# SYSTRAN/faster-whisper

Hardware: AMD Instinct MI355X
Metric: audio-sec/sec (RTF) large-v3 fp16 beam=5 batch=16 (higher is better)
Workload: dtype f16

## Files before the change

faster_whisper_amd/csrc/dec_kernels.hip:

```cpp
#include "common.h"
#include "dec_kernels.h"
#include <stdlib.h>
#include <atomic>
#include <type_traits>

namespace fwd {
static std::atomic<int> g_self_attn_form{0};
static std::atomic<int> g_forms_epoch{0};
static std::atomic<int> g_cross_regs{0};
}

__device__ __forceinline__ size_t frag_off(int row, int k, int KS) {
  return ((size_t)((row >> 4) * KS + (k >> 5)) * 64 + ((k >> 3) & 3) * 16 + (row & 15)) * 8 + (k & 7);
}

static __device__ __forceinline__ int ragged_pos(const int* __restrict__ ptab, int chunk, int step, int reach) {
  const int p = ptab[chunk] - 1 + step;
  return p < reach ? p : reach - 1;
}

__global__ void dec_embed_kernel(const int* __restrict__ tok, const half_t* __restrict__ emb,
                                 const half_t* __restrict__ pos_emb, half_t* __restrict__ x,
                                 half_t* __restrict__ xfrag, int d, const int* __restrict__ d_step, int pos_fixed,
                                 int P, int blk_n, const int* __restrict__ ptab, int kmul, int reach) {
// ... 621 lines not shown
    int rt = rt0 + a; if (rt > n_rt - 1) rt = n_rt - 1;
    xp[a] = reinterpret_cast<const intx4*>(xfv) + (size_t)rt * KS * 64 + lane;
  }
  floatx4 accf[RT][NT];
  intx4 acci[RT][NT];
  float rs[RT], rq[RT];
#pragma unroll
  for (int a = 0; a < RT; ++a) {
    rs[a] = 0.f; rq[a] = 0.f;
#pragma unroll
    for (int b = 0; b < NT; ++b) { accf[a][b] = floatx4{0, 0, 0, 0}; acci[a][b] = intx4{0, 0, 0, 0}; }
  }
  struct Set { intx4 w[CH][NT]; intx4 x[CH][RT]; };
  auto load = [&](Set& f, int ks0) {
#pragma unroll
    for (int j = 0; j < CH; ++j) {
      int ks = ks0 + j; if (ks > KS - 1) ks = KS - 1;
#pragma unroll
      for (int b = 0; b < NT; ++b) f.w[j][b] = wp[b][(size_t)ks * 64];
#pragma unroll
      for (int a = 0; a < RT; ++a) f.x[j][a] = xp[a][(size_t)ks * 64];
    }
  };
  auto compute = [&](const Set& f, int ks0) {
#pragma unroll
    for (int j = 0; j < CH; ++j) {
      if (ks0 + j < KS) {
#pragma unroll
        for (int a = 0; a < RT; ++a) {
#pragma unroll
          for (int b = 0; b < NT; ++b) {
            if (I8) acci[a][b] = __builtin_amdgcn_mfma_i32_16x16x64_i8(f.w[j][b], f.x[j][a], acci[a][b], 0, 0, 0);
            else accf[a][b] = __builtin_amdgcn_mfma_f32_16x16x32_f16(__builtin_bit_cast(half8_t, f.w[j][b]),
                                                                    __builtin_bit_cast(half8_t, f.x[j][a]), accf[a][b],
                                                                    0, 0, 0);
          }
          if (LNF && !SPLIT) {
            const half8_t xv = __builtin_bit_cast(half8_t, f.x[j][a]);
            const half2_t one2 = {(half_t)1.f, (half_t)1.f};
#pragma unroll
            for (int e = 0; e < 4; ++e) {
              const half2_t h2 = {xv[2 * e], xv[2 * e + 1]};
              rs[a] = __builtin_amdgcn_fdot2(h2, one2, rs[a], false);
              rq[a] = __builtin_amdgcn_fdot2(h2, h2, rq[a], false);
            }
          }
        }
        if (SPLIT) {
          const half2_t one2 = {(half_t)1.f, (half_t)1.f};
          const intx4 xsel = wn == 0 ? f.x[j][0] : (wn == 1 ? f.x[j][1] : (wn == 2 ? f.x[j][2] : f.x[j][RT > 3 ? 3 : 0]));
          const half8_t xv = __builtin_bit_cast(half8_t, xsel);
#pragma unroll
          for (int e = 0; e < 4; ++e) {
            const half2_t h2 = {xv[2 * e], xv[2 * e + 1]};
            rs[0] = __builtin_amdgcn_fdot2(h2, one2, rs[0], false);
            rq[0] = __builtin_amdgcn_fdot2(h2, h2, rq[0], false);
          }
          if (RT > 4 && wn == 0) {
            const half8_t xw = __builtin_bit_cast(half8_t, f.x[j][RT > 4 ? 4 : 0]);
#pragma unroll
            for (int e = 0; e < 4; ++e) {
              const half2_t h2 = {xw[2 * e], xw[2 * e + 1]};
              rs[1] = __builtin_amdgcn_fdot2(h2, one2, rs[1], false);
              rq[1] = __builtin_amdgcn_fdot2(h2, h2, rq[1], false);
            }
          }
        }
      }
    }
  };
  float ks1[NT][4], kcf[NT][4], kws[NT][4];
  half_t kb[NT][4];
#pragma unroll
  for (int b = 0; b < NT; ++b) {
#pragma unroll
    for (int e = 0; e < 4; ++e) {
      const int n = (ct0 + b) * 16 + 4 * g + e;
      const int ne = n < N ? n : N - 1;
      ks1[b][e] = kcf[b][e] = 0.f; kws[b][e] = 1.f; kb[b][e] = (half_t)0.f;
      if (I8) kws[b][e] = w_scale[ne];
      if (LNF) { ks1[b][e] = s1[ne]; kcf[b][e] = cf[ne]; }
      else if (bias) kb[b][e] = bias[ne];
    }
  }
  Set fa, fb;
  load(fa, 0);
  for (int ks0 = 0; ks0 < KS; ks0 += 2 * CH) {
    load(fb, ks0 + CH);
    compute(fa, ks0);
    load(fa, ks0 + 2 * CH);
    compute(fb, ks0 + CH);
  }
  if (SPLIT) {
#pragma unroll
    for (int q = 0; q < 2; ++q) {
      if (q == 1 && !(RT > 4 && wn == 0)) break;
      float sa = rs[q], sb = rq[q];
      sa += __shfl_xor(sa, 16, 64); sa += __shfl_xor(sa, 32, 64);
      sb += __shfl_xor(sb, 16, 64); sb += __shfl_xor(sb, 32, 64);
      if (g == 0) { xst[q == 0 ? wn : 4][i][0] = sa; xst[q == 0 ? wn : 4][i][1] = sb; }
    }
    __syncthreads();
  }
#pragma unroll
  for (int a = 0; a < RT; ++a) {
    float mu = 0.f, rstd = 1.f;
    if (LNF) {
      float sa, sb;
      if (SPLIT) {
        sa = xst[a][i][0]; sb = xst[a][i][1];
      } else {
        sa = rs[a]; sb = rq[a];
        sa += __shfl_xor(sa, 16, 64); sa += __shfl_xor(sa, 32, 64);
        sb += __shfl_xor(sb, 16, 64); sb += __shfl_xor(sb, 32, 64);
      }
      mu = sa / (float)K;
      rstd = rsqrtf(fmaxf(sb / (float)K - mu * mu, 0.f) + 1e-5f);
    }
    const int row = (rt0 + a) * 16 + i;
    if (rt0 + a >= n_rt || row >= R) continue;
    const float sx = I8 ? x_scale[row] : 1.f;
    const bool pair_ok = (ldo & 1) == 0;
#pragma unroll
    for (int b = 0; b < NT; ++b) {
      if (ct0 + b >= n_ct) continue;
      const int n = (ct0 + b) * 16 + 4 * g;
      float t4[4];
#pragma unroll
      for (int e = 0; e < 4; ++e) {
        float tv = I8 ? (float)acci[a][b][e] * sx * kws[b][e] : accf[a][b][e];
        if (LNF) tv = rstd * (tv - mu * ks1[b][e]) + kcf[b][e];
        else if (bias) tv += (float)kb[b][e];
        t4[e] = tv;
      }
      if (F32 && pair_ok) {
        float* o = reinterpret_cast<float*>(outv) + (size_t)row * ldo + n;
        if (n + 1 < N) *reinterpret_cast<floatx2*>(o) = floatx2{t4[0], t4[1]};
        else if (n < N) o[0] = t4[0];
        if (n + 3 < N) *reinterpret_cast<floatx2*>(o + 2) = floatx2{t4[2], t4[3]};
        else if (n + 2 < N) o[2] = t4[2];
        continue;
      }
#pragma unroll
      for (int e = 0; e < 4; ++e) {
        if (n + e >= N) continue;
        if (F32) reinterpret_cast<float*>(outv)[(size_t)row * ldo + n + e] = t4[e];
        else reinterpret_cast<half_t*>(outv)[(size_t)row * ldo + n + e] = (half_t)t4[e];
      }
    }
  }
}

#define SA_MAX_CTX 448
static __device__ __forceinline__ float sum8_dpp(float v) {
  v += __builtin_bit_cast(float, __builtin_amdgcn_update_dpp(0, __builtin_bit_cast(int, v), 0xB1, 0xF, 0xF, true));
  v += __builtin_bit_cast(float, __builtin_amdgcn_update_dpp(0, __builtin_bit_cast(int, v), 0x4E, 0xF, 0xF, true));
  v += __builtin_bit_cast(float, __builtin_amdgcn_update_dpp(0, __builtin_bit_cast(int, v), 0x141, 0xF, 0xF, true));
  return v;
}
template <bool RAG = false>
__global__ __launch_bounds__(1024) __attribute__((amdgpu_waves_per_eu(8, 8))) void dec_self_attn_kernel(const half_t* __restrict__ qkv, int d, half_t* __restrict__ kc,
                                                             half_t* __restrict__ vc, int n_ctx, int cache_ctx,
                                                             int H, const uint8_t* __restrict__ kvidx2, int Kbeam, int kmul,
                                                             half_t* __restrict__ out, const int* __restrict__ d_step,
                                                             int pos_fixed, int P, int R_total, int frag,
                                                             const int* __restrict__ ptab, int reach) {
  extern __shared__ float sa_smem[];
  const int lane = threadIdx.x & 63;
  const int wave = __builtin_amdgcn_readfirstlane(threadIdx.x >> 6);
  float* sp = sa_smem + (size_t)wave * 2 * n_ctx;
  int* ssrc = reinterpret_cast<int*>(sp + n_ctx);
  const int h = blockIdx.x, c = blockIdx.y;
  const int r = c * kmul + wave, kb = wave;
  const int step = *d_step;
  const int pos = RAG ? ragged_pos(ptab, c, step, reach) : (pos_fixed >= 0 ? pos_fixed : P - 1 + step);
  const int slot = c * Kbeam + kb;
  const int cur = (pos_fixed >= 0) ? 0 : (step & 1);
  const uint8_t* kvidx = kvidx2 + ((size_t)cur * R_total + slot) * n_ctx;
  const half_t* qr = qkv + (size_t)r * 3 * d + h * 64;
  const size_t head_stride = (size_t)cache_ctx * 64;
  const size_t slot_stride = (size_t)H * head_stride;
  const int pg = lane >> 3, cc = lane & 7;
  const half8_t q8 = *reinterpret_cast<const half8_t*>(qr + cc * 8);
  const half8_t kn8 = *reinterpret_cast<const half8_t*>(qr + d + cc * 8);
  const half8_t vn8 = *reinterpret_cast<const half8_t*>(qr + 2 * d + cc * 8);
  float q[8];
#pragma unroll
  for (int e = 0; e < 8; ++e) q[e] = (float)q8[e] * 0.125f;
  if (pg == 0) {
    *reinterpret_cast<half8_t*>(kc + slot * slot_stride + h * head_stride + (size_t)pos * 64 + cc * 8) = kn8;
    *reinterpret_cast<half8_t*>(vc + slot * slot_stride + h * head_stride + (size_t)pos * 64 + cc * 8) = vn8;
  }
  auto dot8 = [&](const half8_t& k) {
    float sacc = 0.f;
#pragma unroll
    for (int e = 0; e < 8; ++e) sacc += q[e] * (float)k[e];
    return sum8_dpp(sacc);
  };
  const float s_new = dot8(kn8);
  float mx = s_new;
  const half_t* kbase = kc + h * head_stride + cc * 8;
  for (int p0 = 0; p0 < pos; p0 += 32) {
    half8_t kv[4];
    int src[4];
#pragma unroll
    for (int j = 0; j < 4; ++j) {
      const int p = p0 + 8 * j + pg;
      const int pc = p < pos ? p : pos - 1;
      src[j] = c * Kbeam + kvidx[pc];
      kv[j] = *reinterpret_cast<const half8_t*>(kbase + src[j] * slot_stride + (size_t)pc * 64);
    }
#pragma unroll
    for (int j = 0; j < 4; ++j) {
      const int p = p0 + 8 * j + pg;
      const float sc = dot8(kv[j]);
      if (p < pos) {
        if (cc == 0) { sp[p] = sc; ssrc[p] = src[j]; }
        mx = fmaxf(mx, sc);
      }
    }
  }
  mx = wave_max(mx);
  __builtin_amdgcn_wave_barrier();
  float sum = 0.f;
  for (int p = lane; p < pos; p += 64) {
    const float e = __expf(sp[p] - mx);
    sp[p] = e;
    sum += e;
  }
  const float e_new = __expf(s_new - mx);
  sum = wave_sum(sum) + e_new;
  __builtin_amdgcn_wave_barrier();
  float acc[8];
#pragma unroll
  for (int e = 0; e < 8; ++e) acc[e] = 0.f;
  const half_t* vb = vc + h * head_stride + cc * 8;
#pragma unroll 4
  for (int p = pg; p < pos; p += 8) {
    const half8_t vv = *reinterpret_cast<const half8_t*>(vb + ssrc[p] * slot_stride + (size_t)p * 64);
    const float w = sp[p];
#pragma unroll
    for (int e = 0; e < 8; ++e) acc[e] += w * (float)vv[e];
  }
#pragma unroll
  for (int e = 0; e < 8; ++e) {
    float a = acc[e];
    a += __shfl_xor(a, 8, 64);
    a += __shfl_xor(a, 16, 64);
    a += __shfl_xor(a, 32, 64);
    acc[e] = a;
  }
  if (pg == 0) {
    const float inv = 1.f / sum;
    half8_t o;
#pragma unroll
    for (int e = 0; e < 8; ++e) o[e] = (half_t)((acc[e] + e_new * (float)vn8[e]) * inv);
    half_t* dst = frag ? out + frag_off(r, h * 64 + cc * 8, d >> 5) : out + (size_t)r * d + h * 64 + cc * 8;
    *reinterpret_cast<half8_t*>(dst) = o;
  }
}

template <int U, bool PIPE, int MAXT, bool PB = false, bool RAG = false>
__global__ __launch_bounds__(MAXT) void dec_self_attn2_kernel(const half_t* __restrict__ qkv, int d, half_t* __restrict__ kc,
                                                             half_t* __restrict__ vc, int n_ctx, int cache_ctx,
                                                             int H, const uint8_t* __restrict__ kvidx2, int Kbeam, int kmul,
                                                             half_t* __restrict__ out, const int* __restrict__ d_step,
                                                             int pos_fixed, int P, int R_total, int frag,
                                                             const int* __restrict__ ptab, int reach) {
  static_assert(!(PB && RAG), "position blocks take explicit positions");
  extern __shared__ float sa_smem[];
  constexpr int NB = 4 * U;
  const int lane = threadIdx.x & 63;
  const int wave = __builtin_amdgcn_readfirstlane(threadIdx.x >> 6);
  float* sp = sa_smem + (size_t)wave * 2 * n_ctx;
  int* ssrc = reinterpret_cast<int*>(sp + n_ctx);
  const int h = blockIdx.x, c = blockIdx.y;
  const int r = c * kmul + wave, kb = PB ? 0 : wave;
  const int step = PB ? 0 : *d_step;
  const int pos = PB ? pos_fixed + wave
                     : (RAG ? ragged_pos(ptab, c, step, reach) : (pos_fixed >= 0 ? pos_fixed : P - 1 + step));
  const int slot = c * Kbeam + kb;
  const int cur = (pos_fixed >= 0) ? 0 : (step & 1);
  const uint8_t* kvidx = kvidx2 + ((size_t)cur * R_total + slot) * n_ctx;
  const half_t* qr = qkv + (size_t)r * 3 * d + h * 64;
  const size_t head_stride = (size_t)cache_ctx * 64;
  const size_t slot_stride = (size_t)H * head_stride;
  const int pg = lane >> 3, cc = lane & 7;
  for (int p4 = 4 * lane; p4 < pos; p4 += 256) {
    const unsigned w = PB ? 0u : *reinterpret_cast<const unsigned*>(kvidx + p4);
    intx4 s4;
    s4[0] = c * Kbeam + (int)(w & 0xffu); s4[1] = c * Kbeam + (int)((w >> 8) & 0xffu);
    s4[2] = c * Kbeam + (int)((w >> 16) & 0xffu); s4[3] = c * Kbeam + (int)(w >> 24);
    *reinterpret_cast<intx4*>(ssrc + p4) = s4;
  }
  const half8_t q8 = *reinterpret_cast<const half8_t*>(qr + cc * 8);
  const half8_t kn8 = *reinterpret_cast<const half8_t*>(qr + d + cc * 8);
  const half8_t vn8 = *reinterpret_cast<const half8_t*>(qr + 2 * d + cc * 8);
  float q[8];
#pragma unroll
  for (int e = 0; e < 8; ++e) q[e] = (float)q8[e] * 0.125f;
  if (pg == 0) {
    *reinterpret_cast<half8_t*>(kc + slot * slot_stride + h * head_stride + (size_t)pos * 64 + cc * 8) = kn8;
    *reinterpret_cast<half8_t*>(vc + slot * slot_stride + h * head_stride + (size_t)pos * 64 + cc * 8) = vn8;
  }
  auto dot8 = [&](const half8_t& k) {
    float sacc = 0.f;
#pragma unroll
    for (int e = 0; e < 8; ++e) sacc = __builtin_fmaf(q[e], (float)k[e], sacc);
    return sum8_dpp(sacc);
  };
  const float s_new = dot8(kn8);
  float mx = s_new;
  __builtin_amdgcn_wave_barrier();
  const char* kbase = reinterpret_cast<const char*>(kc + h * head_stride);
  const char* vbase = reinterpret_cast<const char*>(vc + h * head_stride);
  const unsigned slot_bytes = (unsigned)(slot_stride * sizeof(half_t));
  struct Batch { half8_t row[NB]; };
  auto fetch = [&](Batch& b, const char* base, int p0, const half_t* sib) {
#pragma unroll
    for (int j = 0; j < NB; ++j) {
      const int p = p0 + 8 * j + pg;
      const int pc = p < pos ? p : pos - 1;
      const unsigned off = (unsigned)ssrc[pc] * slot_bytes + (unsigned)(pc * 128 + cc * 16);
      if (PB && pc >= pos_fixed)
        b.row[j] = *reinterpret_cast<const half8_t*>(sib + (size_t)(pc - pos_fixed) * 3 * d + cc * 8);
      else
        b.row[j] = *reinterpret_cast<const half8_t*>(base + off);
    }
  };
  const half_t* ksib = qkv + (size_t)c * kmul * 3 * d + d + h * 64;
  const half_t* vsib = ksib + d;
  auto score = [&](const Batch& b, int p0) {
#pragma unroll
    for (int j = 0; j < NB; ++j) {
      const int p = p0 + 8 * j + pg;
      const float sc = dot8(b.row[j]);
      if (p < pos) {
        if (cc == 0) sp[p] = sc;
        mx = fmaxf(mx, sc);
      }
    }
  };
  Batch b0, b1;
  if (pos > 0) {
    fetch(b0, kbase, 0, ksib);
    for (int p0 = 0; p0 < pos; p0 += 16 * NB) {
      if (PIPE) {
        fetch(b1, kbase, p0 + 8 * NB, ksib);
        score(b0, p0);
        fetch(b0, kbase, p0 + 16 * NB, ksib);
        score(b1, p0 + 8 * NB);
      } else {
        score(b0, p0);
        if (p0 + 8 * NB < pos) {
          fetch(b0, kbase, p0 + 8 * NB, ksib);
          score(b0, p0 + 8 * NB);
          if (p0 + 16 * NB < pos) fetch(b0, kbase, p0 + 16 * NB, ksib);
        }
      }
    }
    fetch(b0, vbase, 0, vsib);
  }
  mx = wave_max_v(mx);
  __builtin_amdgcn_wave_barrier();
  float sum = 0.f;
  for (int p = lane; p < pos; p += 64) {
    const float e = __expf(sp[p] - mx);
    sp[p] = e;
    sum += e;
  }
  const float e_new = __expf(s_new - mx);
  sum = wave_sum_v(sum) + e_new;
  __builtin_amdgcn_wave_barrier();
  float acc[8];
#pragma unroll
  for (int e = 0; e < 8; ++e) acc[e] = 0.f;
  auto accum = [&](const Batch& b, int p0) {
#pragma unroll
    for (int j = 0; j < NB; ++j) {
      const int p = p0 + 8 * j + pg;
      if (p < pos) {
        const float w = sp[p];
#pragma unroll
        for (int e = 0; e < 8; ++e) acc[e] = __builtin_fmaf(w, (float)b.row[j][e], acc[e]);
      }
    }
  };
  for (int p0 = 0; p0 < pos; p0 += 16 * NB) {
    if (PIPE) {
      fetch(b1, vbase, p0 + 8 * NB, vsib);
      accum(b0, p0);
      fetch(b0, vbase, p0 + 16 * NB, vsib);
      accum(b1, p0 + 8 * NB);
    } else {
      accum(b0, p0);
      if (p0 + 8 * NB < pos) {
        fetch(b0, vbase, p0 + 8 * NB, vsib);
        accum(b0, p0 + 8 * NB);
        if (p0 + 16 * NB < pos) fetch(b0, vbase, p0 + 16 * NB, vsib);
      }
    }
  }
#pragma unroll
  for (int e = 0; e < 8; ++e) acc[e] = sum_x8_x16_x32_v(acc[e]);
  if (pg == 0) {
    const float inv = 1.f / sum;
    half8_t o;
#pragma unroll
    for (int e = 0; e < 8; ++e) o[e] = (half_t)((acc[e] + e_new * (float)vn8[e]) * inv);
    half_t* dst = frag ? out + frag_off(r, h * 64 + cc * 8, d >> 5) : out + (size_t)r * d + h * 64 + cc * 8;
    *reinterpret_cast<half8_t*>(dst) = o;
  }
}

template <int CA_WAVES, bool NTL, int MINW = 1>
__global__ __launch_bounds__(CA_WAVES * 64, MINW) void dec_cross_attn_kernel(const half_t* __restrict__ qx, int d,
                                                             const half_t* __restrict__ ck,
                                                             const half_t* __restrict__ cvt, int T, int kvp,
                                                             int kmul, half_t* __restrict__ out,
                                                             const int* __restrict__ done, int kv_div, int frag,
                                                             const int* __restrict__ slot_map) {
  __shared__ float sm[CA_WAVES][16], sl[CA_WAVES][16];
  __shared__ float so[CA_WAVES][16][65];
  const int h = blockIdx.x, c = blockIdx.y;
  if (done && done[c]) return;
  const int tid = threadIdx.x, lane = tid & 63, wave = tid >> 6;
  const int j = lane & 15, g = lane >> 4;
  const int ce = slot_map[c / kv_div];
  const half_t* kbase = ck + ((size_t)ce * (d >> 6) + h) * kvp * 64 + lane * 8;
  const half_t* vbase = cvt + ((size_t)ce * (d >> 6) + h) * kvp * 64 + lane * 8;
  half8_t qf[2];
  {
    if (j < kmul) {
      const half_t* qp = qx + (size_t)(c * kmul + j) * d + h * 64 + g * 8;
#pragma unroll
      for (int s = 0; s < 2; ++s) {
        half8_t v = *reinterpret_cast<const half8_t*>(qp + s * 32);
#pragma unroll
        for (int e = 0; e < 8; ++e) v[e] = v[e] * (half_t)0.125f;
        qf[s] = v;
      }
    } else {
      qf[0] = half8_t{0, 0, 0, 0, 0, 0, 0, 0};
      qf[1] = qf[0];
    }
  }
  floatx4 o[4];
#pragma unroll
  for (int dt = 0; dt < 4; ++dt) o[dt] = floatx4{0, 0, 0, 0};
  float m_run = -1.0e30f, l_run = 0.f;
  const float LOG2E = 1.4426950408889634f;
  const int ngroups = (T + 31) >> 5;
  auto load_kv = [&](int gi, half8_t (&kf)[4], half8_t (&vf)[4]) {
    const half_t* kp = kbase + (size_t)gi * 2048;
    const half_t* vp = vbase + (size_t)gi * 2048;
#pragma unroll
    for (int q = 0; q < 4; ++q)
      kf[q] = NTL ? __builtin_nontemporal_load(reinterpret_cast<const half8_t*>(kp + q * 512))
                  : *reinterpret_cast<const half8_t*>(kp + q * 512);
#pragma unroll
    for (int dt = 0; dt < 4; ++dt)
      vf[dt] = NTL ? __builtin_nontemporal_load(reinterpret_cast<const half8_t*>(vp + dt * 512))
                   : *reinterpret_cast<const half8_t*>(vp + dt * 512);
  };
  half8_t kcur[4], vcur[4], knxt[4], vnxt[4];
  if (wave < ngroups) load_kv(wave, kcur, vcur);
  for (int gi = wave; gi < ngroups; gi += CA_WAVES) {
    const int base = gi * 32;
    const bool has_next = (gi + CA_WAVES) < ngroups;
    if (has_next) load_kv(gi + CA_WAVES, knxt, vnxt);
    floatx4 s0 = {0, 0, 0, 0}, s1 = {0, 0, 0, 0};
    s0 = __builtin_amdgcn_mfma_f32_16x16x32_f16(kcur[0], qf[0], s0, 0, 0, 0);
    s0 = __builtin_amdgcn_mfma_f32_16x16x32_f16(kcur[1], qf[1], s0, 0, 0, 0);
    s1 = __builtin_amdgcn_mfma_f32_16x16x32_f16(kcur[2], qf[0], s1, 0, 0, 0);
    s1 = __builtin_amdgcn_mfma_f32_16x16x32_f16(kcur[3], qf[1], s1, 0, 0, 0);
    float sc[8];
    float mx = -1.0e30f;
#pragma unroll
    for (int e = 0; e < 8; ++e) {
      float v = (e < 4 ? s0[e] : s1[e - 4]) * LOG2E;
      if (base + 8 * g + e >= T) v = -1.0e30f;
      sc[e] = v;
      mx = fmaxf(mx, v);
    }
    mx = pair16_max(mx);
    mx = pair32_max(mx);
    const float m_new = fmaxf(m_run, mx);
    const float alpha = __builtin_amdgcn_exp2f(m_run - m_new);
    m_run = m_new;
    half8_t pf;
    float psum = 0.f;
#pragma unroll
    for (int e = 0; e < 8; ++e) {
      const float pv = __builtin_amdgcn_exp2f(sc[e] - m_new);
      psum += pv;
      pf[e] = (half_t)pv;
    }
    l_run = l_run * alpha + psum;
#pragma unroll
    for (int dt = 0; dt < 4; ++dt) {
#pragma unroll
      for (int e = 0; e < 4; ++e) o[dt][e] *= alpha;
      o[dt] = __builtin_amdgcn_mfma_f32_16x16x32_f16(vcur[dt], pf, o[dt], 0, 0, 0);
    }
    if (has_next) {
#pragma unroll
      for (int q = 0; q < 4; ++q) { kcur[q] = knxt[q]; vcur[q] = vnxt[q]; }
    }
  }
  l_run = pair16_sum(l_run);
  l_run = pair32_sum(l_run);
  if (g == 0) { sm[wave][j] = m_run; sl[wave][j] = l_run; }
#pragma unroll
  for (int dt = 0; dt < 4; ++dt)
#pragma unroll
    for (int e = 0; e < 4; ++e) so[wave][j][dt * 16 + 4 * g + e] = o[dt][e];
  __syncthreads();
  for (int idx = tid; idx < kmul * 64; idx += CA_WAVES * 64) {
    const int qq = idx >> 6, dh = idx & 63;
    float M = sm[0][qq];
#pragma unroll
    for (int w = 1; w < CA_WAVES; ++w) M = fmaxf(M, sm[w][qq]);
    float Lsum = 0.f, O = 0.f;
#pragma unroll
    for (int w = 0; w < CA_WAVES; ++w) {
      const float f = __builtin_amdgcn_exp2f(sm[w][qq] - M);
      Lsum += sl[w][qq] * f;
      O += so[w][qq][dh] * f;
    }
    const int orow = c * kmul + qq;
    half_t* dst = frag ? out + frag_off(orow, h * 64 + dh, d >> 5) : out + (size_t)orow * d + h * 64 + dh;
    *dst = (half_t)(O / Lsum);
  }
}

template <bool RAG, bool ALT = false>
__global__ __launch_bounds__(64) __attribute__((amdgpu_waves_per_eu(8, 8)))
void dec_beam_update_kernel(fwd::GenDev gp, const int* __restrict__ ptab, const float* __restrict__ cand_val,
                                                             const int* __restrict__ cand_tok, int* __restrict__ hist2,
                                                             float* __restrict__ cum2, uint8_t* __restrict__ kvidx2,
                                                             int* __restrict__ cur_tok, const int* __restrict__ d_step,
                                                             int* __restrict__ done, int* __restrict__ n_done,
                                                             int* __restrict__ n_fin, int* __restrict__ fin_tok,
                                                             int* __restrict__ fin_len, float* __restrict__ fin_score,
                                                             float* __restrict__ fin_cum,
                                                             const float* __restrict__ cand_lp,
                                                             float* __restrict__ lphist2, float* __restrict__ fin_lp,
                                                             uint8_t* __restrict__ fin_path) {
  __shared__ float ov[32], olp[32];
  __shared__ int ok[32], ot[32];
  __shared__ int s_parent[16], s_tok[16];
  __shared__ float s_cum[16], s_lp[16];
  __shared__ int s_done;
  const int c = blockIdx.x;
  if (done[c]) return;
  const int tid = threadIdx.x;
  const int K = gp.K, C = 2 * K, NT = gp.n_text_ctx;
  const int step = *d_step;
  const int cur = step & 1, nxt = cur ^ 1;
  const int Pc = RAG ? ptab[c] : gp.P;
  const int pos = Pc - 1 + step;
  const bool last_step = (step + 1) >= (RAG ? gp.reach - Pc : gp.budget);
// ... 216 lines not shown

#define DL_ARGS a.xf, a.Wf, a.bias, a.s1, a.cf, a.res, a.ldr, a.out, a.ldo, a.out_frag, a.R, a.N, a.K, a.act
template <bool LNF, int RT, int NT, int CH = 0>
static void frag_go(hipStream_t st, int waves, const DecLin& a) {
  const dim3 grid((a.N / 16 + NT - 1) / NT, ((a.R + 15) / 16 + RT - 1) / RT);
  if (waves == 8) dec_gemm_frag_kernel<8, LNF, RT, NT, CH><<<grid, 512, 0, st>>>(DL_ARGS);
  else dec_gemm_frag_kernel<4, LNF, RT, NT, CH><<<grid, 256, 0, st>>>(DL_ARGS);
}

template <bool LNF, int S, int WM, int WN, int FB, int KC, int NST>
static int big_go(hipStream_t st, const DecLin& a) {
  constexpr int lds = (4 * WM + FB * WN) * KC * 1024 * NST;
  static std::atomic<unsigned long long> attr_done{0};
  int dev = 0;
  (void)hipGetDevice(&dev);
  if (!((attr_done.load(std::memory_order_acquire) >> (dev & 63)) & 1ull)) {
    if (hipFuncSetAttribute(reinterpret_cast<const void*>(dec_gemm_big_kernel<LNF, S, WM, WN, FB, KC, NST>),
                            hipFuncAttributeMaxDynamicSharedMemorySize, lds) != hipSuccess)
      return -1;
    attr_done.fetch_or(1ull << (dev & 63), std::memory_order_release);
  }
  const int nMt = ((a.R + 15) / 16 + 4 * WM - 1) / (4 * WM), nNt = (a.N / 16 + FB * WN - 1) / (FB * WN);
  dec_gemm_big_kernel<LNF, S, WM, WN, FB, KC, NST><<<nMt * nNt, WM * WN * 64, lds, st>>>(DL_ARGS, nNt);
  return hipPeekAtLastError() == hipSuccess ? 0 : -1;
}
template <int CFG>
static int big_cfg(hipStream_t st, int slices, const DecLin& a) {
  constexpr BigShape b = BIG_SHAPES[CFG];
#define DGB(LNF_, S_) big_go<LNF_, S_, b.WM, b.WN, b.FB, b.KC, b.NST>(st, a)
  if (a.s1) return slices == 8 ? DGB(true, 8) : DGB(true, 4);
  return slices == 8 ? DGB(false, 8) : DGB(false, 4);
#undef DGB
}

int launch_dec_linear(hipStream_t st, const DecLin& a, int form) {
  const DecLinPlan p = dec_linear_plan(a.R, a.N, a.K, a.ldo, a.res ? a.ldr : 0, 0, form);
  if (p.family == DEC_LIN_FAMILY_BIG) {
    int rc = -1;
    switch (p.cfg) {
      case 0: rc = big_cfg<0>(st, p.waves, a); break;
      case 1: rc = big_cfg<1>(st, p.waves, a); break;
      case 2: rc = big_cfg<2>(st, p.waves, a); break;
    }
    return rc == 0 || form != DEC_LIN_PRODUCT ? rc : launch_dec_linear(st, a, DEC_LIN_SKINNY);
  }
  if (p.family != DEC_LIN_FAMILY_SKINNY) return -1;
  if (p.row_tiles == 1) {
    if (a.s1) frag_go<true, 1, 1, 10>(st, p.waves, a);
    else frag_go<false, 1, 1, 10>(st, p.waves, a);
  } else {
    if (a.s1) frag_go<true, 2, 2>(st, p.waves, a);
    else frag_go<false, 2, 2>(st, p.waves, a);
  }
  return 0;
}
#undef DL_ARGS

template <int WAVES, int RT, int NT, int CH>
static void frag_variant(hipStream_t st, bool lnf, const half_t* xf, const half_t* Wf, const half_t* bias,
                         const float* s1, const float* cf, half_t* out, int R, int N, int K) {
  const dim3 grid(N / 16 / NT, ((R + 15) / 16 + RT - 1) / RT);
  if (lnf)
    dec_gemm_frag_kernel<WAVES, true, RT, NT, CH><<<grid, WAVES * 64, 0, st>>>(xf, Wf, bias, s1, cf, nullptr, 0, out, N,
                                                                              nullptr, R, N, K, 0);
  else
    dec_gemm_frag_kernel<WAVES, false, RT, NT, CH><<<grid, WAVES * 64, 0, st>>>(xf, Wf, bias, nullptr, nullptr, nullptr,
                                                                               0, out, N, nullptr, R, N, K, 0);
}
int launch_dec_gemm_frag_variant(hipStream_t st, int variant, bool lnf, const half_t* xf, const half_t* Wf,
                                 const half_t* bias, const float* s1, const float* cf, half_t* out, int R, int N,
                                 int K) {
  if (K % 32 != 0 || N % 64 != 0 || R < 1) return -1;
  switch (variant) {
    case 0: frag_variant<4, 2, 2, 5>(st, lnf, xf, Wf, bias, s1, cf, out, R, N, K); break;
    case 1: frag_variant<8, 2, 2, 5>(st, lnf, xf, Wf, bias, s1, cf, out, R, N, K); break;
    case 2: frag_variant<8, 4, 2, 3>(st, lnf, xf, Wf, bias, s1, cf, out, R, N, K); break;
    case 3: frag_variant<8, 4, 2, 4>(st, lnf, xf, Wf, bias, s1, cf, out, R, N, K); break;
    case 4: frag_variant<8, 4, 4, 2>(st, lnf, xf, Wf, bias, s1, cf, out, R, N, K); break;
    case 5: frag_variant<8, 4, 4, 3>(st, lnf, xf, Wf, bias, s1, cf, out, R, N, K); break;
    case 6: frag_variant<4, 4, 2, 3>(st, lnf, xf, Wf, bias, s1, cf, out, R, N, K); break;
    case 7: frag_variant<8, 2, 4, 3>(st, lnf, xf, Wf, bias, s1, cf, out, R, N, K); break;
    case 8: frag_variant<8, 8, 2, 2>(st, lnf, xf, Wf, bias, s1, cf, out, R, N, K); break;
    case 9: frag_variant<4, 4, 4, 2>(st, lnf, xf, Wf, bias, s1, cf, out, R, N, K); break;
    case 23: frag_variant<4, 1, 1, 10>(st, lnf, xf, Wf, bias, s1, cf, out, R, N, K); break;
    case 24: frag_variant<8, 1, 1, 10>(st, lnf, xf, Wf, bias, s1, cf, out, R, N, K); break;
    case 25: frag_variant<4, 1, 2, 6>(st, lnf, xf, Wf, bias, s1, cf, out, R, N, K); break;
    case 26: frag_variant<8, 1, 2, 6>(st, lnf, xf, Wf, bias, s1, cf, out, R, N, K); break;
    case 21: frag_variant<4, 4, 4, 5>(st, lnf, xf, Wf, bias, s1, cf, out, R, N, K); break;
    case 22: frag_variant<8, 4, 4, 5>(st, lnf, xf, Wf, bias, s1, cf, out, R, N, K); break;
    case 10: case 11: case 12:
      return launch_dec_linear(st, DecLin{xf, Wf, lnf ? nullptr : bias, lnf ? s1 : nullptr, lnf ? cf : nullptr, nullptr, 0,
                                          out, N, nullptr, R, N, K, 0}, variant);
    default: return -1;
  }
  return 0;
}

int launch_dec_gemm_frag_i8(hipStream_t st, const int8_t* xq, const float* x_scale, const int8_t* Wq,
                            const float* w_scale, const half_t* bias, const half_t* res, int ldr, half_t* out, int ldo,
                            int R, int N, int K, int act) {
  const DecLinPlan p = dec_linear_plan(R, N, K, ldo, res ? ldr : 0, 1, DEC_LIN_PRODUCT);
  if (p.family != DEC_LIN_FAMILY_SKINNY || !x_scale || !w_scale) return -1;
  const dim3 grid(N / 16 / p.col_tiles, ((R + 15) / 16 + p.row_tiles - 1) / p.row_tiles);
#define I8_ARGS xq, x_scale, Wq, w_scale, bias, res, ldr, out, ldo, R, N, K, act
  if (p.row_tiles == 4) {
    if (p.waves == 8) dec_gemm_frag_i8_kernel<8, 4, 4, 3><<<grid, 512, 0, st>>>(I8_ARGS);
    else dec_gemm_frag_i8_kernel<4, 4, 4, 5><<<grid, 256, 0, st>>>(I8_ARGS);
  } else {
    if (p.waves == 8) dec_gemm_frag_i8_kernel<8, 2, 2><<<grid, 512, 0, st>>>(I8_ARGS);
    else dec_gemm_frag_i8_kernel<4, 2, 2><<<grid, 256, 0, st>>>(I8_ARGS);
  }
#undef I8_ARGS
  return 0;
}

template <bool I8, bool LNF, int RT>
static void wave_go(hipStream_t st, const void* xf, const float* x_scale, const void* Wf, const float* w_scale,
                    const float* s1, const float* cf, float* out, int ldo, int R, int N, int K) {
  constexpr int NT = 2, WM = 1, WN = 4;
  const int n_rt = (R + 15) / 16, n_ct = (N + 15) / 16;
  const int n_cg = ((n_ct + NT * WN - 1) / (NT * WN) + 7) & ~7;
  const int n_rg = (n_rt + RT * WM - 1) / (RT * WM);
  dec_gemm_wave_kernel<I8, LNF, true, RT, NT, WM, WN><<<n_cg * n_rg, WM * WN * 64, 0, st>>>(
      xf, x_scale, Wf, w_scale, nullptr, s1, cf, out, ldo, R, N, K, n_rg);
}

int launch_dec_logits(hipStream_t st, bool i8, const void* xf, const float* x_scale, const void* Wf,
                      const float* w_scale, const float* s1, const float* cf, float* out, int ldo, int R, int N, int K) {
  if (K % (i8 ? 64 : 32) != 0 || R < 1) return -1;
  if (i8 ? (!x_scale || !w_scale) : ((s1 == nullptr) != (cf == nullptr))) return -1;
  const int n_rt = (R + 15) / 16;
#define WG(RT)                                                                                   \
  do {                                                                                           \
    if (i8) wave_go<true, false, RT>(st, xf, x_scale, Wf, w_scale, s1, cf, out, ldo, R, N, K);   \
    else if (s1) wave_go<false, true, RT>(st, xf, x_scale, Wf, w_scale, s1, cf, out, ldo, R, N, K); \
    else wave_go<false, false, RT>(st, xf, x_scale, Wf, w_scale, s1, cf, out, ldo, R, N, K);     \
  } while (0)
  if (n_rt == 1) WG(1);
  else if (n_rt == 2) WG(2);
  else if (n_rt == 3) WG(3);
  else if (n_rt == 4) WG(4);
  else WG(5);
#undef WG
  return 0;
}

bool self_attn_block_ok(int n_ctx, int cache_ctx, int d, int R_total) {
  return (n_ctx & 3) == 0 && (size_t)R_total * cache_ctx * d * sizeof(half_t) < ((size_t)1 << 32);
}

int self_attn_form(int n_ctx, int cache_ctx, int d, int R_total, int kmul, int H, int chunks, int knob) {
  if (knob == 1 || !self_attn_block_ok(n_ctx, cache_ctx, d, R_total)) return 1;
  if (knob == 0) return kmul <= 8 && H * chunks <= 768 ? 2 : 3;
  return knob == 2 && kmul <= 8 ? 2 : 3;
}

void launch_self_attn(hipStream_t st, const half_t* qkv, int d, half_t* kc, half_t* vc, int n_ctx, int cache_ctx, int H,
                      const uint8_t* kvidx2, int Kbeam, int kmul, half_t* out, int rows, const int* d_step,
                      int pos_fixed, int P, int R_total, int frag, int blk_n, const int* ptab, int reach) {
  if (blk_n > 0) {
    dec_self_attn2_kernel<1, true, 1024, true><<<dim3(H, rows / blk_n), blk_n * 64, (size_t)blk_n * 2 * n_ctx * sizeof(float), st>>>(
        qkv, d, kc, vc, n_ctx, cache_ctx, H, kvidx2, Kbeam, blk_n, out, d_step, pos_fixed, P, R_total, frag, nullptr, 0);
    return;
  }
  if (pos_fixed >= 0) ptab = nullptr;
  const dim3 grid(H, rows / kmul);
  const size_t lds = (size_t)kmul * 2 * n_ctx * sizeof(float);
  const int form = self_attn_form(n_ctx, cache_ctx, d, R_total, kmul, H, rows / kmul,
                                  g_self_attn_form.load(std::memory_order_relaxed));
#define SA_ARGS qkv, d, kc, vc, n_ctx, cache_ctx, H, kvidx2, Kbeam, kmul, out, d_step, pos_fixed, P, R_total, frag, ptab, reach
  if (ptab) {
    if (form == 1) dec_self_attn_kernel<true><<<grid, kmul * 64, lds, st>>>(SA_ARGS);
    else if (form == 2) dec_self_attn2_kernel<4, false, 512, false, true><<<grid, kmul * 64, lds, st>>>(SA_ARGS);
    else dec_self_attn2_kernel<1, true, 1024, false, true><<<grid, kmul * 64, lds, st>>>(SA_ARGS);
  }
  else if (form == 1) dec_self_attn_kernel<false><<<grid, kmul * 64, lds, st>>>(SA_ARGS);
  else if (form == 2) dec_self_attn2_kernel<4, false, 512><<<grid, kmul * 64, lds, st>>>(SA_ARGS);
  else dec_self_attn2_kernel<1, true, 1024><<<grid, kmul * 64, lds, st>>>(SA_ARGS);
#undef SA_ARGS
}
void set_self_attn_form(int form) { g_self_attn_form.store(form); g_forms_epoch.fetch_add(1); }
int kernel_forms_epoch() { return g_forms_epoch.load(); }
void bump_kernel_forms_epoch() { g_forms_epoch.fetch_add(1); }

void launch_cross_attn(hipStream_t st, const half_t* qx, int d, const half_t* ck, const half_t* cvt, int T, int kvp,
                       int kmul, half_t* out, int B, int H, const int* done, int kv_div, int frag, const int* slot_map) {
  const int cap = g_cross_regs.load(std::memory_order_relaxed);
  if (cap == 1)
    dec_cross_attn_kernel<8, true, 5><<<dim3(H, B), 512, 0, st>>>(qx, d, ck, cvt, T, kvp, kmul, out, done, kv_div, frag, slot_map);
  else if (cap == 2)
    dec_cross_attn_kernel<8, true, 6><<<dim3(H, B), 512, 0, st>>>(qx, d, ck, cvt, T, kvp, kmul, out, done, kv_div, frag, slot_map);
  else
    dec_cross_attn_kernel<8, true><<<dim3(H, B), 512, 0, st>>>(qx, d, ck, cvt, T, kvp, kmul, out, done, kv_div, frag, slot_map);
}
void set_cross_attn_regs(int cap) { g_cross_regs.store(cap); g_forms_epoch.fetch_add(1); }

void launch_beam_update(hipStream_t st, const GenDev& gp, const float* cand_val, const int* cand_tok, int* hist2,
                        float* cum2, uint8_t* kvidx2, int* cur_tok, const int* d_step, int* done, int* n_done,
                        int* n_fin, int* fin_tok, int* fin_len, float* fin_score, float* fin_cum, const float* cand_lp,
                        float* lphist2, float* fin_lp, const int* ptab, uint8_t* fin_path) {
  if (!cand_lp || !lphist2 || !fin_lp) { cand_lp = nullptr; lphist2 = nullptr; fin_lp = nullptr; }
#define BU_ARGS gp, ptab, cand_val, cand_tok, hist2, cum2, kvidx2, cur_tok, d_step, done, n_done, n_fin, fin_tok, fin_len, \
                fin_score, fin_cum, cand_lp, lphist2, fin_lp, fin_path
  if (fin_path) {
    if (ptab) dec_beam_update_kernel<true, true><<<gp.B, 64, 0, st>>>(BU_ARGS);
    else dec_beam_update_kernel<false, true><<<gp.B, 64, 0, st>>>(BU_ARGS);
  } else if (ptab) dec_beam_update_kernel<true, false><<<gp.B, 64, 0, st>>>(BU_ARGS);
  else dec_beam_update_kernel<false, false><<<gp.B, 64, 0, st>>>(BU_ARGS);
#undef BU_ARGS
}

__global__ __launch_bounds__(256) void dec_alt_gather_kernel(const int* __restrict__ alt_tok, const float* __restrict__ alt_lp,
                                                             const uint8_t* __restrict__ fin_path,
                                                             const fwd::AltHyp* __restrict__ hyps, int R, int K, int NT,
                                                             int n_alt, int T, int* __restrict__ out_tok,
                                                             float* __restrict__ out_lp) {
  const fwd::AltHyp h = hyps[blockIdx.x];
  const uint8_t* path = fin_path + ((size_t)h.chunk * fwd::FIN_CAP + h.fin) * (NT + 1);
  const size_t o0 = (size_t)blockIdx.x * (T + 1) * n_alt;
  for (int i = threadIdx.x; i < (T + 1) * n_alt; i += blockDim.x) {
    const int t = i / n_alt, j = i - t * n_alt;
    const int q = t < T ? (t < h.len ? t : -1) : h.end;
    int tok = -1;
    float lp = 0.f;
    if (q >= 0) {
      const size_t src = ((size_t)q * R + h.chunk * K + path[q]) * n_alt + j;
      tok = alt_tok[src];
      lp = alt_lp[src];
    }
    out_tok[o0 + i] = tok;
    out_lp[o0 + i] = lp;
  }
}

void launch_alt_gather(hipStream_t st, const int* alt_tok, const float* alt_lp, const uint8_t* fin_path, const AltHyp* hyps,
                       int n_hyp, int R, int K, int NT, int n_alt, int T, int* out_tok, float* out_lp) {
  if (n_hyp <= 0) return;
  dec_alt_gather_kernel<<<n_hyp, 256, 0, st>>>(alt_tok, alt_lp, fin_path, hyps, R, K, NT, n_alt, T, out_tok, out_lp);
}

__global__ void dec_gather_sot_rows_kernel(const half_t* __restrict__ x, const int* __restrict__ sot_tab,
                                           const int* __restrict__ ptab, int pos0, int nb, int rows_per_chunk,
                                           half_t* __restrict__ xo, half_t* __restrict__ xof, int d) {
  const int c = blockIdx.x;
  const int sp = sot_tab[c], last = ptab[c] - 1;
  int src;
  if (nb > 0) {
    if (sp < pos0 || sp >= pos0 + nb || sp >= last) return;
    src = c * nb + (sp - pos0);
  } else {
    if (sp != last) return;
    src = c * rows_per_chunk;
  }
  const half2_t* xi = reinterpret_cast<const half2_t*>(x + (size_t)src * d);
  half2_t* o = reinterpret_cast<half2_t*>(xo + (size_t)c * d);
  for (int i = threadIdx.x; i < d / 2; i += blockDim.x) {
    const half2_t v = xi[i];
    o[i] = v;
    *reinterpret_cast<half2_t*>(xof + frag_off(c, 2 * i, d >> 5)) = v;
  }
}

void launch_gather_sot_rows(hipStream_t st, const half_t* x, const int* sot_tab, const int* ptab, int pos0, int nb,
                            int rows_per_chunk, half_t* xo, half_t* xof, int d, int B) {
  dec_gather_sot_rows_kernel<<<B, 128, 0, st>>>(x, sot_tab, ptab, pos0, nb, rows_per_chunk, xo, xof, d);
}

void launch_step_advance(hipStream_t st, int* d_step) { dec_step_advance_kernel<<<1, 1, 0, st>>>(d_step); }

void launch_cross_probs(hipStream_t st, const half_t* qx, int d, const half_t* ck, int T, int kvp, const int* heads,
                        int n_layer_heads, int n_sel, float* probs, int n_tok, int tok_idx, int B, int blk_n) {
  const int bn = blk_n > 0 ? blk_n : 1;
  dec_cross_probs_kernel<<<dim3(n_layer_heads, B * bn), 256, 0, st>>>(qx, d, ck, T, kvp, heads, n_sel, probs, n_tok,
                                                                      tok_idx, bn);
}

}
```

Measured before the change: 3175.

## Add specialized short-context self-attention path with unified K/V prefetch pipeline

```diff
diff --git a/faster_whisper_amd/csrc/dec_kernels.hip b/faster_whisper_amd/csrc/dec_kernels.hip
--- a/faster_whisper_amd/csrc/dec_kernels.hip
+++ b/faster_whisper_amd/csrc/dec_kernels.hip
@@ -797,6 +797,10 @@
 }
 
 #define SA_MAX_CTX 448
+static __device__ __forceinline__ size_t sgpr_u64(size_t a) {
+  const unsigned lo = __builtin_amdgcn_readfirstlane((unsigned)a), hi = __builtin_amdgcn_readfirstlane((unsigned)(a >> 32));
+  return ((size_t)hi << 32) | lo;
+}
 static __device__ __forceinline__ float sum8_dpp(float v) {
   v += __builtin_bit_cast(float, __builtin_amdgcn_update_dpp(0, __builtin_bit_cast(int, v), 0xB1, 0xF, 0xF, true));
   v += __builtin_bit_cast(float, __builtin_amdgcn_update_dpp(0, __builtin_bit_cast(int, v), 0x4E, 0xF, 0xF, true));
@@ -905,8 +909,8 @@
   }
 }
 
-template <int U, bool PIPE, int MAXT, bool PB = false, bool RAG = false>
-__global__ __launch_bounds__(MAXT) void dec_self_attn2_kernel(const half_t* __restrict__ qkv, int d, half_t* __restrict__ kc,
+template <int U, bool PIPE, int MAXT, bool PB = false, bool RAG = false, bool SPEC = false>
+__global__ __launch_bounds__(MAXT) __attribute__((amdgpu_waves_per_eu(SPEC ? 7 : 1, 8))) void dec_self_attn2_kernel(const half_t* __restrict__ qkv, int d, half_t* __restrict__ kc,
                                                              half_t* __restrict__ vc, int n_ctx, int cache_ctx,
                                                              int H, const uint8_t* __restrict__ kvidx2, int Kbeam, int kmul,
                                                              half_t* __restrict__ out, const int* __restrict__ d_step,
@@ -930,7 +934,7 @@
   const half_t* qr = qkv + (size_t)r * 3 * d + h * 64;
   const size_t head_stride = (size_t)cache_ctx * 64;
   const size_t slot_stride = (size_t)H * head_stride;
-  const int pg = lane >> 3, cc = lane & 7;
+  int pg = lane >> 3, cc = lane & 7;
   for (int p4 = 4 * lane; p4 < pos; p4 += 256) {
     const unsigned w = PB ? 0u : *reinterpret_cast<const unsigned*>(kvidx + p4);
     intx4 s4;
@@ -986,6 +990,113 @@
       }
     }
   };
+  auto vnew_again = [&](int cc_) {
+    const half_t* vr = qr + 2 * d + cc_ * 8;
+    asm volatile("" : "+v"(vr));
+    return *reinterpret_cast<const half8_t*>(vr);
+  };
+  if constexpr (SPEC) {
+    static_assert(U == 1 && PIPE && !PB, "the throughput form");
+    const size_t head_bytes = sgpr_u64(h * head_stride * sizeof(half_t));
+    const char* kb_s = reinterpret_cast<const char*>(kc) + head_bytes;
+    const char* vb_s = reinterpret_cast<const char*>(vc) + head_bytes;
+    int pos_v = pos;
+    asm volatile("" : "+s"(pos_v));
+    auto body = [&](auto nbk_c) {
+      constexpr int NBK = decltype(nbk_c)::value;
+      int ln = lane;
+      asm volatile("" : "+v"(ln));
+      const int pg = ln >> 3, cc = ln & 7;
+      Batch bb[2];
+      auto fetch_s = [&](int i) {
+        const char* base = i < NBK ? kb_s : vb_s;
+        const int k = i < NBK ? i : i - NBK;
+        const int pe = i < NBK ? pos : pos_v;
+#pragma unroll
+        for (int j = 0; j < NB; ++j) {
+          const int p = 32 * k + 8 * j + pg;
+          const int pc = (k == NBK - 1 && p >= pe) ? pe - 1 : p;
+          const unsigned off = (unsigned)ssrc[pc] * slot_bytes + (unsigned)((pc - 32 * k) * 128 + cc * 16);
+          bb[i & 1].row[j] = *reinterpret_cast<const half8_t*>(base + 4096 * k + off);
+        }
+      };
+      fetch_s(0);
+      fetch_s(1);
+      __builtin_amdgcn_sched_barrier(0);
+#pragma unroll
+      for (int k = 0; k < NBK; ++k) {
+#pragma unroll
+        for (int j = 0; j < NB; ++j) {
+          const int p = 32 * k + 8 * j + pg;
+          const float sc = dot8(bb[k & 1].row[j]);
+          if (k < NBK - 1 || p < pos) {
+            if (cc == 0) sp[p] = sc;
+            mx = fmaxf(mx, sc);
+          }
+        }
+        __builtin_amdgcn_sched_barrier(0);
+        if (k + 2 < 2 * NBK) fetch_s(k + 2);
+        __builtin_amdgcn_sched_barrier(0);
+      }
+      mx = wave_max_v(mx);
+      __builtin_amdgcn_wave_barrier();
+      float sum = 0.f;
+      constexpr int NR = (NBK + 1) / 2;
+#pragma unroll
+      for (int i = 0; i < NR; ++i) {
+        const int p = ln + 64 * i;
+        if (i < NR - 1 || p < pos) {
+          const float e = __expf(sp[p] - mx);
+          sp[p] = e;
+          sum += e;
+        }
+      }
+      const float e_new = __expf(s_new - mx);
+      sum = wave_sum_v(sum) + e_new;
+      __builtin_amdgcn_wave_barrier();
+      float acc[8];
+#pragma unroll
+      for (int e = 0; e < 8; ++e) acc[e] = 0.f;
+#pragma unroll
+      for (int k = 0; k < NBK; ++k) {
+#pragma unroll
+        for (int j = 0; j < NB; ++j) {
+          const int p = 32 * k + 8 * j + pg;
+          if (k < NBK - 1 || p < pos) {
+            const float w = sp[p];
+#pragma unroll
+            for (int e = 0; e < 8; ++e) acc[e] = __builtin_fmaf(w, (float)bb[(NBK + k) & 1].row[j][e], acc[e]);
+          }
+        }
+        asm volatile("" : "+v"(acc[0]), "+v"(acc[1]), "+v"(acc[2]), "+v"(acc[3]), "+v"(acc[4]), "+v"(acc[5]), "+v"(acc[6]),
+                          "+v"(acc[7]) :: "memory");
+        __builtin_amdgcn_sched_barrier(0);
+        if (k + 2 < NBK) fetch_s(NBK + k + 2);
+        __builtin_amdgcn_sched_barrier(0);
+      }
+#pragma unroll
+      for (int e = 0; e < 8; ++e) acc[e] = sum_x8_x16_x32_v(acc[e]);
+      if (pg == 0) {
+        const half8_t vn = vnew_again(cc);
+        const float inv = 1.f / sum;
+        half8_t o;
+#pragma unroll
+        for (int e = 0; e < 8; ++e) o[e] = (half_t)((acc[e] + e_new * (float)vn[e]) * inv);
+        half_t* dst = frag ? out + frag_off(r, h * 64 + cc * 8, d >> 5) : out + (size_t)r * d + h * 64 + cc * 8;
+        *reinterpret_cast<half8_t*>(dst) = o;
+      }
+    };
+    switch ((pos + 31) >> 5) {
+      case 1: body(std::integral_constant<int, 1>{}); return;
+      case 2: body(std::integral_constant<int, 2>{}); return;
+      case 3: body(std::integral_constant<int, 3>{}); return;
+      case 4: body(std::integral_constant<int, 4>{}); return;
+      default: break;
+    }
+    int ll = lane;
+    asm volatile("" : "+v"(ll));
+    pg = ll >> 3; cc = ll & 7;
+  }
   Batch b0, b1;
   if (pos > 0) {
     fetch(b0, kbase, 0, ksib);
@@ -1049,10 +1160,11 @@
 #pragma unroll
   for (int e = 0; e < 8; ++e) acc[e] = sum_x8_x16_x32_v(acc[e]);
   if (pg == 0) {
+    const half8_t vn = SPEC ? vnew_again(cc) : vn8;
     const float inv = 1.f / sum;
     half8_t o;
 #pragma unroll
-    for (int e = 0; e < 8; ++e) o[e] = (half_t)((acc[e] + e_new * (float)vn8[e]) * inv);
+    for (int e = 0; e < 8; ++e) o[e] = (half_t)((acc[e] + e_new * (float)vn[e]) * inv);
     half_t* dst = frag ? out + frag_off(r, h * 64 + cc * 8, d >> 5) : out + (size_t)r * d + h * 64 + cc * 8;
     *reinterpret_cast<half8_t*>(dst) = o;
   }
@@ -1575,6 +1687,7 @@
 int self_attn_form(int n_ctx, int cache_ctx, int d, int R_total, int kmul, int H, int chunks, int knob) {
   if (knob == 1 || !self_attn_block_ok(n_ctx, cache_ctx, d, R_total)) return 1;
   if (knob == 0) return kmul <= 8 && H * chunks <= 768 ? 2 : 3;
+  if (knob == 4) return 4;
   return knob == 2 && kmul <= 8 ? 2 : 3;
 }
 
@@ -1595,11 +1708,13 @@
   if (ptab) {
     if (form == 1) dec_self_attn_kernel<true><<<grid, kmul * 64, lds, st>>>(SA_ARGS);
     else if (form == 2) dec_self_attn2_kernel<4, false, 512, false, true><<<grid, kmul * 64, lds, st>>>(SA_ARGS);
-    else dec_self_attn2_kernel<1, true, 1024, false, true><<<grid, kmul * 64, lds, st>>>(SA_ARGS);
+    else if (form == 4) dec_self_attn2_kernel<1, true, 1024, false, true><<<grid, kmul * 64, lds, st>>>(SA_ARGS);
+    else dec_self_attn2_kernel<1, true, 1024, false, true, true><<<grid, kmul * 64, lds, st>>>(SA_ARGS);
   }
   else if (form == 1) dec_self_attn_kernel<false><<<grid, kmul * 64, lds, st>>>(SA_ARGS);
   else if (form == 2) dec_self_attn2_kernel<4, false, 512><<<grid, kmul * 64, lds, st>>>(SA_ARGS);
-  else dec_self_attn2_kernel<1, true, 1024><<<grid, kmul * 64, lds, st>>>(SA_ARGS);
+  else if (form == 4) dec_self_attn2_kernel<1, true, 1024><<<grid, kmul * 64, lds, st>>>(SA_ARGS);
+  else dec_self_attn2_kernel<1, true, 1024, false, false, true><<<grid, kmul * 64, lds, st>>>(SA_ARGS);
 #undef SA_ARGS
 }
 void set_self_attn_form(int form) { g_self_attn_form.store(form); g_forms_epoch.fetch_add(1); }
```

After: 3179, median of 6. About the same (+0.1%).
